# liuzuxin/FSRL

Measured on AMD Instinct MI355X. Metric: policy-updates/sec (PPO-Lagrangian update(), SafetyCarCircle-v0 shape, 256x256 MLP, 20k-step buffer), higher is better.
Workload: dtype f32; 1 GPU; configs[1] PPO-Lag update: repeat 4, clip 0.5, KL stop off, batch 256, N=20000 (20x1000), obs 8/act 2, 256x256; seeds_per_gpu=1, parallelism=independent agents x1

## Files before the change

### fsrl_amd/csrc/common.hpp

```cpp
#pragma once
#include <hip/hip_runtime.h>
#include <stdint.h>

#include "../../include/fsrl_hip.h"

#define FSRL_MAX_NETS (1 + FSRL_MAX_CRITICS)
#define FSRL_TILE_M 16
#define FSRL_DOW 32
#define FSRL_MAX_OBS 128
#define FSRL_MAX_ACT 16
#define FSRL_W1_LDS 16
#define FSRL_RD 64
#define FSRL_RD_LOGP 16
#define FSRL_RD_ADV 17
#define FSRL_RD_RET 21
#define FSRL_RD_VOLD 25
#define FSRL_RD_MEAN 32
#define FSRL_RD_STD 48

typedef float f32x4 __attribute__((ext_vector_type(4)));
typedef float f32x2 __attribute__((ext_vector_type(2)));

struct NetOff {
    int sigma;
// ... 33 lines not shown
    float rescale;
    float lam[FSRL_MAX_CRITICS];
    float eps_clip, dual_clip, vf_coef, max_action, max_grad_norm, target_kl;
    int norm_adv, use_lagrangian;
    float lr, beta1, beta2, adam_eps;
    float one_minus_b1, one_minus_b2;
    double kl_thresh;
    float step_size;
    float bc2_sqrt;
    int value_clip;
    int fuse_adam;
    int xcd_pair;
    int dbg_phase;
};
#ifdef FSRL_PROBES
#define FSRL_PROBE(sa, n) ((sa).dbg_phase == (n))
#define FSRL_TS(buf, k) do { if ((buf) && threadIdx.x == 0) (buf)[(size_t)blockIdx.x * 16 + (k)] = __builtin_readcyclecounter(); } while (0)
#else
#define FSRL_PROBE(sa, n) false
#define FSRL_TS(buf, k) do { } while (0)
#endif

__device__ __forceinline__ void ppo_adam_math(const float g, float& m, float& v, float& p, const PpoStepArgs& sa) {
#pragma clang fp contract(off)
    m = fmaf(sa.one_minus_b1, g - m, m);
    v = v * sa.beta2;
    v = fmaf(sa.one_minus_b2 * g, g, v);
    const float denom = sqrtf(v) / sa.bc2_sqrt + sa.adam_eps;
    p = p + (-sa.step_size * m) / denom;
}

struct CtrlBlock {
    int stopped_after;
    int pad;
    double kl_sum;
    float last_grad_norm;
    float pad2;
};

__device__ __forceinline__ f32x4 mfma_16x16x4(float a, float b, f32x4 c) {
    return __builtin_amdgcn_mfma_f32_16x16x4f32(a, b, c, 0, 0, 0);
}

__device__ __forceinline__ f32x4 mfma_4x4x1(float a, float b, f32x4 c) {
    return __builtin_amdgcn_mfma_f32_4x4x1f32(a, b, c, 0, 0, 0);
}

__device__ __forceinline__ void store4_next(float* p, const f32x4 v) {
    asm volatile("global_store_dwordx4 %0, %1, off sc1\n\ts_nop 1" ::"v"(p), "v"(v) : "memory");
}
#ifdef FSRL_FB_PLAIN_STORES
__device__ __forceinline__ void store4_fb(float* p, const f32x4 v) { *reinterpret_cast<f32x4*>(p) = v; }
#else
__device__ __forceinline__ void store4_fb(float* p, const f32x4 v) { store4_next(p, v); }
#endif

__host__ __device__ __forceinline__ unsigned div_magic(const int d) { return d > 1 ? 0xFFFFFFFFu / (unsigned)d + 1u : 0u; }
__device__ __forceinline__ int div_by_magic(const unsigned e, const unsigned magic) { return magic ? (int)__umulhi(e, magic) : (int)e; }

#ifndef WG3_NO_BUFFER
typedef unsigned wg3_u32x4 __attribute__((ext_vector_type(4)));
struct Wg3Buf { __amdgpu_buffer_rsrc_t r; };
__device__ __forceinline__ Wg3Buf wg3_buf(const float* base) {
    Wg3Buf b; b.r = __builtin_amdgcn_make_buffer_rsrc(const_cast<float*>(base), 0, 0x7FFFFFFF, 0x00020000); return b;
}
__device__ __forceinline__ Wg3Buf wg3_buf_here(const float* base) {
    unsigned long long p = (unsigned long long)base;
// ... 37 lines not shown
```

### fsrl_amd/csrc/fsrl_hip.hip

```cpp
#include <hip/hip_runtime.h>

#include <climits>
#include <cstddef>
#include <cmath>
#include <cstdarg>
#include <cstdio>
#include <cstdlib>
#include <cstring>
#include <algorithm>
#include <functional>
#include <queue>
#include <string>
#include <vector>

#include "kernels_misc.hpp"
#include "kernels_mlp.hpp"
#include "kernels_fb.hpp"
#include "kernels_fbco.hpp"
#include "kernels_wgrad2.hpp"
#include "kernels_wgrad3.hpp"
#include "kernels_layered.hpp"
#include "kernels_focops_group.hpp"

static thread_local std::string g_err;
// ... 55 lines not shown
    struct CommState* comm = nullptr;
    int device = 0;
    hipStream_t compute = nullptr, side = nullptr;
    ModelDesc md{};
    std::vector<TensorMap> tmap;
    int h1 = 0, h2 = 0;
    int64_t n_api = 0;
    int n_dev = 0;
    int n_alloc = 0;
    float *P = nullptr, *M = nullptr, *V = nullptr, *G = nullptr;
    int64_t adam_t = 0;
    CtrlBlock* ctrl = nullptr;
    CtrlBlock* h_ctrl = nullptr;
    bool verdict_pending = false;

    int64_t sub_size = 0, maxsize = 0;
    float* mbstat = nullptr; size_t mbstat_cap = 0;
    double* d_rms = nullptr;
    double* ret64 = nullptr; int64_t ret64_cap = 0;
    int64_t alloc_rows = 0;
    int active_envs = 0;
    std::vector<EnvBook> env;
    std::vector<uint8_t> h_flags;
    StorePtrs st{};
    static constexpr int STAGE_CAP = 4096;
    Staging stage[2];
    int cur_stage = 0;
    hipEvent_t store_ready = nullptr;

    BatchPtrs b{};
    int* d_indices = nullptr; uint8_t* d_end = nullptr; int* d_seg = nullptr;
    int* h_indices = nullptr; uint8_t* h_end = nullptr; int* h_seg = nullptr;
    float *values = nullptr, *vnext = nullptr, *advs = nullptr, *rets = nullptr, *logp_old = nullptr;
    int64_t N = 0;
    int n_seg = 0;
    bool batch_ready = false;

    int batch_size = 0, mbp_max = 0, n_tiles_max = 0;
    float *A1 = nullptr, *A2 = nullptr, *D1 = nullptr, *D2 = nullptr, *DO = nullptr;
    float *obs_p = nullptr, *rd_p = nullptr;
    float *statp = nullptr, *gsq_part = nullptr;
    int *d_perm = nullptr, *h_perm = nullptr;
    int *d_mbstart = nullptr, *d_mbsize = nullptr, *h_mbplan = nullptr;
    size_t mb_cap = 0;
    std::vector<int> mb_start, mb_size;
    float* d_stats = nullptr; int64_t stats_cap = 0;
    int64_t n_steps = 0;
    int pass_index = 0;
    double lagr[FSRL_MAX_CRITICS] = {0, 0, 0, 0};
    double rescaling = 1.0;
    bool in_update = false;

    void* scratch = nullptr; size_t scratch_bytes = 0;

    bool profiling = false;
    hipEvent_t ev_a = nullptr, ev_b = nullptr, ev_c = nullptr;
    std::vector<hipEvent_t> k_ev;
    size_t k_ev_used = 0;
    double t_process_ms = 0, t_learn_ms = 0, t_fwdbwd_ms = 0, t_fwdbwd_raw_ms = 0;
    int64_t n_fwdbwd = 0;
    uint64_t rng[4] = {0x9E3779B97F4A7C15ull, 0xBF58476D1CE4E5B9ull, 0x94D049BB133111EBull, 1};
    uint64_t shuffle_rng[4] = {0xD6E8FEB86659FD93ull, 0xA0761D6478BD642Full, 0xE7037ED1A0B428DBull, 2};
    struct Parts { int stride = 0; float* p = nullptr; size_t floats = 0; } parts[3];
    float* wg_parts = nullptr;
    int n_cus = 256;
    bool wgrad_xcd = false;
// ... 227 lines not shown
    for (int net = 0; net < md.n_nets; ++net) {
        const NetOff& no = md.net[net];
        for (int n = 0; n < H; ++n)
            for (int k = 0; k < H; ++k) v[(size_t)no.W2f + w2f_index(H, n, k)] = v[(size_t)no.W2 + (size_t)n * H + k];
    }
}

extern "C" int fsrl_ctx_destroy(fsrl_ctx* c) {
    if (!c) return 0;
    (void)hipSetDevice(c->device);
    pactor_release(c);
    (void)hipDeviceSynchronize();
    if (c->group) group_detach(c);
    if (c->sac_group) sac_group_detach(c);
    if (c->cvpo_group) cvpo_group_detach(c);
    comm_free(c);
    tr_free(c);
    sac_free(c);
    foc_free(c);
    lay_free(c);
    if (c->h_actor) (void)hipHostFree(c->h_actor);
    if (c->h_done) (void)hipHostFree(c->h_done);
    if (c->h_pa) (void)hipHostFree(c->h_pa);
    if (c->mbstat) (void)hipFree(c->mbstat);
    if (c->d_rms) (void)hipFree(c->d_rms);
    if (c->ret64) (void)hipFree(c->ret64);
    if (c->mu_old) (void)hipFree(c->mu_old);
    if (c->sigma_old) (void)hipFree(c->sigma_old);
    if (c->snap) (void)hipFree(c->snap);
    void* dptrs[] = {c->P, c->M, c->V, c->G, c->ctrl, c->st.obs, c->st.obs_next, c->st.act, c->st.rew,
                     c->st.cost, c->st.flags, c->b.obs, c->b.obs_next, c->b.act, c->b.rew, c->b.cost,
                     c->b.flags, c->d_indices, c->d_end, c->d_seg, c->values, c->vnext, c->advs,
                     c->rets, c->logp_old, c->A1, c->A2, c->D1, c->D2, c->DO, c->obs_p, c->rd_p, c->statp,
                     c->gsq_part, c->d_perm, c->d_mbstart, c->d_mbsize, c->d_stats,
                     c->scratch};
    for (void* p : dptrs) if (p) (void)hipFree(p);
    for (auto& pp : c->parts) if (pp.p) (void)hipFree(pp.p);
    void* hptrs[] = {c->h_ctrl, c->h_indices, c->h_end, c->h_seg, c->h_perm, c->h_mbplan};
    for (void* p : hptrs) if (p) (void)hipHostFree(p);
    for (auto& s : c->stage) {
        if (s.h) (void)hipHostFree(s.h);
        if (s.d) (void)hipFree(s.d);
        if (s.done) (void)hipEventDestroy(s.done);
    }
    for (hipEvent_t e : {c->store_ready, c->ev_a, c->ev_b, c->ev_c, c->perm_copied}) if (e) (void)hipEventDestroy(e);
    for (hipEvent_t e : c->k_ev) (void)hipEventDestroy(e);
    if (c->compute) (void)hipStreamDestroy(c->compute);
    if (c->side) (void)hipStreamDestroy(c->side);
    delete c;
    return 0;
}

extern "C" int fsrl_ctx_create(int device_id, const fsrl_config* cfg, fsrl_ctx** out) {
    CHECK_ARG(cfg && out, "null argument");
    CHECK_ARG(cfg->algo == FSRL_ALGO_PPO_LAG || cfg->algo == FSRL_ALGO_SAC_LAG || cfg->algo == FSRL_ALGO_CPO ||
                  cfg->algo == FSRL_ALGO_TRPO_LAG || cfg->algo == FSRL_ALGO_FOCOPS, "unknown algo %d", cfg->algo);
    CHECK_ARG(cfg->obs_dim >= 1 && cfg->obs_dim <= FSRL_MAX_OBS, "obs_dim must be in [1,%d]", FSRL_MAX_OBS);
    CHECK_ARG(cfg->act_dim >= 1 && cfg->act_dim <= FSRL_MAX_ACT, "act_dim must be in [1,%d]", FSRL_MAX_ACT);
    CHECK_ARG(cfg->n_hidden >= 0 && cfg->n_hidden <= FSRL_MAX_HIDDEN, "n_hidden must be in [0, %d]", FSRL_MAX_HIDDEN);
    bool layered = false;
    int n_hid1 = cfg->hidden1, n_hid2 = cfg->hidden2;
    if (cfg->n_hidden > 0) {
        CHECK_ARG(cfg->hidden1 == 0 && cfg->hidden2 == 0, "give hidden_sizes[n_hidden] or hidden1 / hidden2, not both");
        for (int l = 0; l < cfg->n_hidden; ++l)
            CHECK_ARG(cfg->hidden_sizes[l] >= 1 && cfg->hidden_sizes[l] <= FSRL_MAX_WIDTH, "hidden_sizes[%d] = %d outside [1, %d]", l,
                      cfg->hidden_sizes[l], FSRL_MAX_WIDTH);
        if (cfg->n_hidden == 2 && cfg->hidden_sizes[0] <= 256 && cfg->hidden_sizes[1] <= 256 && !cfg->force_layered) {
// ... 53 lines not shown
    TRY(hipStreamCreateWithFlags(&c->compute, hipStreamNonBlocking));
    TRY(hipStreamCreateWithFlags(&c->side, hipStreamNonBlocking));
    const size_t pb = (size_t)c->n_dev * sizeof(float);
    TRY(hipMalloc(&c->P, (size_t)c->n_alloc * sizeof(float))); TRY(hipMemsetAsync(c->P, 0, (size_t)c->n_alloc * sizeof(float), c->compute));
    TRY(hipMalloc(&c->M, pb)); TRY(hipMalloc(&c->V, pb)); TRY(hipMalloc(&c->G, pb));
    TRY(hipMemsetAsync(c->M, 0, pb, c->compute)); TRY(hipMemsetAsync(c->V, 0, pb, c->compute)); TRY(hipMemsetAsync(c->G, 0, pb, c->compute));
    TRY(hipMalloc(&c->ctrl, sizeof(CtrlBlock)));
    if (cfg->rew_norm) {
        TRY(hipMalloc(&c->d_rms, 3 * FSRL_MAX_CRITICS * sizeof(double)));
        double init[3 * FSRL_MAX_CRITICS];
        for (int i = 0; i < FSRL_MAX_CRITICS; ++i) { init[3 * i] = 0.0; init[3 * i + 1] = 1.0; init[3 * i + 2] = 0.0; }
        TRY(hipMemcpy(c->d_rms, init, sizeof(init), hipMemcpyHostToDevice));
    }
    TRY(hipHostMalloc(&c->h_ctrl, sizeof(CtrlBlock)));
    c->sub_size = (cfg->buffer_size + cfg->env_num - 1) / cfg->env_num;
    c->maxsize = c->sub_size * cfg->env_num;
    c->alloc_rows = c->maxsize + cfg->env_num; c->active_envs = cfg->env_num;
    c->env.resize(cfg->env_num);
    c->h_flags.assign((size_t)c->alloc_rows, 0);
    const size_t ms = (size_t)c->alloc_rows;
    const int Do = cfg->obs_dim, Da = cfg->act_dim;
    TRY(hipMalloc(&c->st.obs, ms * Do * 4)); TRY(hipMalloc(&c->st.obs_next, ms * Do * 4));
    TRY(hipMalloc(&c->st.act, ms * Da * 4)); TRY(hipMalloc(&c->st.rew, ms * 8));
    TRY(hipMalloc(&c->st.cost, ms * 8)); TRY(hipMalloc(&c->st.flags, ms));
    TRY(hipMalloc(&c->b.obs, ms * Do * 4)); TRY(hipMalloc(&c->b.obs_next, ms * Do * 4));
    TRY(hipMalloc(&c->b.act, ms * Da * 4)); TRY(hipMalloc(&c->b.rew, ms * 8));
    TRY(hipMalloc(&c->b.cost, ms * 8)); TRY(hipMalloc(&c->b.flags, ms));
    TRY(hipMalloc(&c->d_indices, ms * 4)); TRY(hipMalloc(&c->d_end, ms)); TRY(hipMalloc(&c->d_seg, (ms + 2) * 4));
    TRY(hipHostMalloc(&c->h_indices, ms * 4)); TRY(hipHostMalloc(&c->h_end, ms)); TRY(hipHostMalloc(&c->h_seg, (ms + 2) * 4));
    const int C = cfg->n_critics;
    TRY(hipMalloc(&c->values, ms * C * 4)); TRY(hipMalloc(&c->vnext, ms * C * 4));
    TRY(hipMalloc(&c->advs, ms * C * 4)); TRY(hipMalloc(&c->rets, ms * C * 4));
    TRY(hipMalloc(&c->logp_old, ms * 4));
    TRY(hipMalloc(&c->d_perm, ms * 4)); TRY(hipHostMalloc(&c->h_perm, ms * 4));
    TRY(hipMalloc(&c->obs_p, (ms + 32) * Do * 4)); TRY(hipMemsetAsync(c->obs_p, 0, (ms + 32) * Do * 4, c->compute));
    TRY(hipMalloc(&c->rd_p, (ms + 32) * FSRL_RD * 4)); TRY(hipMemsetAsync(c->rd_p, 0, (ms + 32) * FSRL_RD * 4, c->compute));
    TRY(hipStreamSynchronize(c->compute));
    for (auto& s : c->stage) {
        const size_t k = fsrl_ctx::STAGE_CAP;
        TRY(hipHostMalloc(&s.h, k * stage_rec_bytes(Do, Da)));
        TRY(hipMalloc(&s.d, k * stage_rec_bytes(Do, Da)));
        TRY(hipEventCreateWithFlags(&s.done, hipEventDisableTiming));
    }
    TRY(hipEventCreateWithFlags(&c->store_ready, hipEventDisableTiming));
    TRY(hipEventCreate(&c->ev_a)); TRY(hipEventCreate(&c->ev_b)); TRY(hipEventCreate(&c->ev_c));
    TRY(hipEventCreateWithFlags(&c->perm_copied, hipEventDisableTiming));
    CtrlBlock init{INT_MAX, 0, 0.0, 0.0f, 0.0f};
    TRY(hipMemcpy(c->ctrl, &init, sizeof(init), hipMemcpyHostToDevice));
#undef TRY
    *out = c;
    return 0;
}

extern "C" int fsrl_sync(fsrl_ctx* c) {
    CHECK_ARG(c, "null ctx");
    ENTER_DEV(c);
    HIPCHK(hipStreamSynchronize(c->side));
    HIPCHK(hipStreamSynchronize(c->compute));
    return 0;
}

extern "C" int64_t fsrl_param_count(const fsrl_ctx* c) { return c ? c->n_api : 0; }

static int copy_flat(fsrl_ctx* c, float* dev, float* host_out, const float* host_in, int64_t n) {
    CHECK_ARG(n == c->n_api, "expected %lld parameters, got %lld", (long long)c->n_api, (long long)n);
    ENTER_DEV(c);
// ... 229 lines not shown
    }
    return 0;
}

extern "C" int fsrl_store_read(fsrl_ctx* c, const int64_t* indices, int64_t n, float* obs_out, float* act_out,
                               double* rew_out, double* cost_out, uint8_t* terminated_out, uint8_t* truncated_out,
                               float* obs_next_out) {
    CHECK_ARG(c && (indices || n == 0), "null argument");
    CHECK_ARG(n >= 0 && n <= c->maxsize, "bad row count");
    if (n == 0) return 0;
    ENTER_DEV(c);
    int rc = join_store(c);
    if (rc) return rc;
    const size_t N = (size_t)n, Do = (size_t)c->cfg.obs_dim, Da = (size_t)c->cfg.act_dim;
    auto al = [](size_t x) { return (x + 255) / 256 * 256; };
    const size_t o_idx = 0, o_end = o_idx + al(N * 4), o_obs = o_end + al(N), o_nxt = o_obs + al(N * Do * 4),
                 o_act = o_nxt + al(N * Do * 4), o_rew = o_act + al(N * Da * 4), o_cost = o_rew + al(N * 8),
                 o_fl = o_cost + al(N * 8), total = o_fl + al(N);
    rc = ensure_scratch(c, total);
    if (rc) return rc;
    std::vector<int> idx(N);
    for (size_t i = 0; i < N; ++i) {
        CHECK_ARG(indices[i] >= 0 && indices[i] < c->maxsize, "index %lld out of range", (long long)indices[i]);
        idx[i] = (int)indices[i];
    }
    char* base = (char*)c->scratch;
    hipStream_t s = c->compute;
    HIPCHK(hipMemcpyAsync(base + o_idx, idx.data(), N * 4, hipMemcpyHostToDevice, s));
    HIPCHK(hipMemsetAsync(base + o_end, 0, N, s));
    BatchPtrs b{(float*)(base + o_obs), (float*)(base + o_nxt), (float*)(base + o_act), (double*)(base + o_rew),
                (double*)(base + o_cost), (uint8_t*)(base + o_fl)};
    const size_t work = N * (2 * Do + Da + 1);
    hipLaunchKernelGGL(batch_gather_kernel, dim3((int)std::min<size_t>(2048, (work + 255) / 256)), dim3(256), 0, s, c->st, b,
                       (const int*)(base + o_idx), (const uint8_t*)(base + o_end), (int)n, (int)Do, (int)Da);
    HIPCHK(hipGetLastError());
    std::vector<uint8_t> fl(N);
    if (obs_out) HIPCHK(hipMemcpyAsync(obs_out, b.obs, N * Do * 4, hipMemcpyDeviceToHost, s));
    if (obs_next_out) HIPCHK(hipMemcpyAsync(obs_next_out, b.obs_next, N * Do * 4, hipMemcpyDeviceToHost, s));
    if (act_out) HIPCHK(hipMemcpyAsync(act_out, b.act, N * Da * 4, hipMemcpyDeviceToHost, s));
    if (rew_out) HIPCHK(hipMemcpyAsync(rew_out, b.rew, N * 8, hipMemcpyDeviceToHost, s));
    if (cost_out) HIPCHK(hipMemcpyAsync(cost_out, b.cost, N * 8, hipMemcpyDeviceToHost, s));
    HIPCHK(hipMemcpyAsync(fl.data(), b.flags, N, hipMemcpyDeviceToHost, s));
    HIPCHK(hipStreamSynchronize(s));
    for (size_t i = 0; i < N; ++i) {
        if (terminated_out) terminated_out[i] = fl[i] & 1;
        if (truncated_out) truncated_out[i] = (fl[i] >> 1) & 1;
    }
    return 0;
}

template <typename F>
static int dispatch_H(int H, F&& f) {
    switch (H) {
        case 64: return f(std::integral_constant<int, 64>());
        case 128: return f(std::integral_constant<int, 128>());
        case 256: return f(std::integral_constant<int, 256>());
    }
    return fail(FSRL_EINVAL, "unsupported hidden width %d", H);
}

static int launch_infer(fsrl_ctx* c, const InferArgs& ia, int jobs_y, hipStream_t s) {
    const int tiles = (ia.N + 15) / 16;
    if (tiles == 0) return 0;
    if (c->lay) return lay_infer(c, ia, jobs_y, s);
    return dispatch_H(c->cfg.hidden, [&](auto hc) {
        constexpr int H = decltype(hc)::value;
        const int gx = std::min(tiles, std::max(1, c->n_cus / jobs_y));
        hipLaunchKernelGGL(mlp_infer_kernel<H>, dim3(gx, jobs_y), dim3(4 * H), 0, s, c->P, c->md, ia);
        HIPCHK(hipGetLastError());
        return 0;
    });
}

struct SacState;
static bool ctx_is_replay(const fsrl_ctx* c) { return c->cfg.algo == FSRL_ALGO_SAC_LAG; }
static int sac_actor_launch(fsrl_ctx* c, const float* h_obs, float* h_raw, int k);
static void sac_actor_finish(fsrl_ctx* c, const float* h_raw, int k, float* mu_out, float* sigma_out);
static int sac_raw_cols(const fsrl_ctx* c);
static bool sac_squashes(fsrl_ctx* c);
static bool sac_actor_resident_args(fsrl_ctx* c, const float** P, const ModelDesc** md);

struct PaLayout { unsigned long long* bell; unsigned* done; unsigned* state; float* obs; float* mu; float* sp; };
static PaLayout pa_layout(const fsrl_ctx* c) {
    char* b = (char*)c->h_pa;
    PaLayout l;
    l.bell = (unsigned long long*)b; l.done = (unsigned*)(b + 16); l.state = (unsigned*)(b + 32);
    l.obs = (float*)(b + 64);
    l.mu = l.obs + (size_t)c->pa_cap * c->cfg.obs_dim;
    l.sp = l.mu + (size_t)c->pa_cap * 2 * c->cfg.act_dim;
    return l;
}

static bool pactor_ok(const fsrl_ctx* c, int k) {
    const int blocks = std::min(PACTOR_BLOCKS, std::max(1, (c->cfg.env_num + 15) / 16));
    if (!(c->pa_on && !c->no_spin && !c->lay && !c->group && k >= 1 && k <= 16 * blocks)) return false;
    if (c->cfg.algo != FSRL_ALGO_SAC_LAG) return true;
    const float* P; const ModelDesc* md;
    return sac_actor_resident_args(const_cast<fsrl_ctx*>(c), &P, &md);
}

static void pactor_release(fsrl_ctx* c) {
// ... 528 lines not shown
```

### fsrl_amd/csrc/host_ppo.inc

```
static int launch_gae(fsrl_ctx* c);
static void split_plan(int n, int B, std::vector<int>& st, std::vector<int>& sz) {
    st.clear(); sz.clear();
    const bool merge = (n % B) > 0;
    for (int i = 0; i < n; i += B) {
        if (merge && i + 2 * B >= n) { st.push_back(i); sz.push_back(n - i); break; }
        st.push_back(i); sz.push_back(std::min(B, n - i));
    }
}

static int ensure_ppo_buffers(fsrl_ctx* c, int B) {
    const int mbp = round_up(2 * B, 32);
    if (mbp <= c->mbp_max) return 0;
    HIPCHK(hipStreamSynchronize(c->compute));
    for (float** p : {&c->A1, &c->A2, &c->D1, &c->D2, &c->DO, &c->statp, &c->gsq_part})
        if (*p) { HIPCHK(hipFree(*p)); *p = nullptr; }
    const int H = c->cfg.hidden, nn = c->md.n_nets;
    const size_t act = (size_t)nn * mbp * H * 4;
    HIPCHK(hipMalloc(&c->A1, act)); HIPCHK(hipMalloc(&c->A2, act));
    HIPCHK(hipMalloc(&c->D1, act)); HIPCHK(hipMalloc(&c->D2, act));
    HIPCHK(hipMalloc(&c->DO, (size_t)nn * mbp * FSRL_DOW * 4));
    HIPCHK(hipMalloc(&c->statp, (size_t)(mbp / 4) * nn * 4 * 4));
    HIPCHK(hipMalloc(&c->gsq_part, (size_t)std::max(wg_grid(H, nn), c->n_dev / 256 + 2) * 4));
    c->mbp_max = mbp;
    c->n_tiles_max = mbp / 16;
// ... 21 lines not shown
    for (int i = 0; i < FSRL_MAX_CRITICS; ++i) c->lagr[i] = 0.0;
    if (c->cfg.use_lagrangian && C > 1) {
        CHECK_ARG(lagrangians, "lags and values length must be equal");
        for (int i = 0; i < C - 1; ++i) c->lagr[i] = lagrangians[i];
    }
    c->rescaling = rescaling;
    c->batch_size = batch_size;
    const int64_t n = sample0(c, c->h_indices, c->h_end);
    c->N = n;
    if (n_out) *n_out = n;
    c->n_steps = 0;
    c->pass_index = 0;
    c->in_update = true;
    c->verdict_pending = false;
    c->t_fwdbwd_ms = 0; c->n_fwdbwd = 0; c->k_ev_used = 0;
    CtrlBlock init{INT_MAX, 0, 0.0, 0.0f, 0.0f};
    *c->h_ctrl = init;
    hipStream_t s = c->compute;
    HIPCHK(hipMemcpyAsync(c->ctrl, c->h_ctrl, sizeof(CtrlBlock), hipMemcpyHostToDevice, s));
    if (n == 0) { c->batch_ready = true; return 0; }
    int nseg = 0;
    c->h_seg[nseg++] = 0;
    for (int64_t i = 0; i + 1 < n; ++i) if (c->h_end[i]) c->h_seg[nseg++] = (int)i + 1;
    c->h_seg[nseg] = (int)n;
    HIPCHK(hipEventRecord(c->ev_a, s));
    HIPCHK(hipMemcpyAsync(c->d_indices, c->h_indices, (size_t)n * 4, hipMemcpyHostToDevice, s));
    HIPCHK(hipMemcpyAsync(c->d_end, c->h_end, (size_t)n, hipMemcpyHostToDevice, s));
    HIPCHK(hipMemcpyAsync(c->d_seg, c->h_seg, (size_t)(nseg + 1) * 4, hipMemcpyHostToDevice, s));
    const int Do = c->cfg.obs_dim, Da = c->cfg.act_dim;
    {
        const size_t work = (size_t)n * (2 * Do + Da + 1);
        const int blocks = (int)std::min<size_t>(2048, (work + 255) / 256);
        hipLaunchKernelGGL(batch_gather_kernel, dim3(blocks), dim3(256), 0, s, c->st, c->b, c->d_indices,
                           c->d_end, (int)n, Do, Da);
        HIPCHK(hipGetLastError());
    }
    InferArgs ia{};
    ia.obs = c->b.obs; ia.obs_next = c->b.obs_next; ia.act = c->b.act; ia.flags = c->b.flags;
    ia.values = c->values; ia.vnext = c->vnext; ia.logp_old = c->logp_old; ia.mu_out = nullptr;
    if (c->cfg.algo == FSRL_ALGO_FOCOPS) {
        if (!c->mu_old) {
            HIPCHK(hipMalloc(&c->mu_old, (size_t)c->alloc_rows * Da * 4));
            HIPCHK(hipMalloc(&c->sigma_old, FSRL_MAX_ACT * 4));
        }
        ia.mu_out = c->mu_old;
        HIPCHK(hipMemcpyAsync(c->sigma_old, c->P + c->md.net[0].sigma, (size_t)Da * 4, hipMemcpyDeviceToDevice, s));
    }
    ia.N = (int)n; ia.C = C; ia.max_action = c->cfg.max_action;
    rc = launch_infer(c, ia, 2 * C + 1, s);
    if (rc) return rc;
    c->n_seg = nseg;
    rc = launch_gae(c);
    if (rc) return rc;
    HIPCHK(hipEventRecord(c->ev_b, s));
    split_plan((int)n, batch_size, c->mb_start, c->mb_size);
    const int bs_rows = (int)std::min<int64_t>(batch_size, std::max<int64_t>(n, 1));
    rc = c->lay ? lay_ensure_mb(c, bs_rows) : ensure_ppo_buffers(c, bs_rows);
    if (rc) return rc;
    const size_t nmb = c->mb_start.size();
    if (nmb > c->mb_cap) {
        HIPCHK(hipStreamSynchronize(s));
        if (c->d_mbstart) HIPCHK(hipFree(c->d_mbstart));
        if (c->d_mbsize) HIPCHK(hipFree(c->d_mbsize));
        if (c->h_mbplan) HIPCHK(hipHostFree(c->h_mbplan));
        c->d_mbstart = c->d_mbsize = nullptr; c->h_mbplan = nullptr;
        const size_t cap = nmb * 2;
        HIPCHK(hipMalloc(&c->d_mbstart, cap * 4)); HIPCHK(hipMalloc(&c->d_mbsize, cap * 4));
        HIPCHK(hipHostMalloc(&c->h_mbplan, cap * 2 * 4));
        c->mb_cap = cap;
    }
    memcpy(c->h_mbplan, c->mb_start.data(), nmb * 4);
    memcpy(c->h_mbplan + c->mb_cap, c->mb_size.data(), nmb * 4);
    HIPCHK(hipMemcpyAsync(c->d_mbstart, c->h_mbplan, nmb * 4, hipMemcpyHostToDevice, s));
    HIPCHK(hipMemcpyAsync(c->d_mbsize, c->h_mbplan + c->mb_cap, nmb * 4, hipMemcpyHostToDevice, s));
    c->batch_ready = true;
    return 0;
}


static int launch_gae(fsrl_ctx* c) {
    GaeArgs ga{};
    ga.values = c->values; ga.vnext = c->vnext; ga.rew = c->b.rew; ga.cost = c->b.cost; ga.flags = c->b.flags;
    ga.seg_start = c->d_seg; ga.advs = c->advs; ga.rets = c->rets; ga.adv64 = nullptr; ga.N = (int)c->N;
    ga.gamma = c->cfg.gamma; ga.gl = c->cfg.gamma * c->cfg.gae_lambda;
    if (c->cfg.rew_norm) {
        if (c->ret64_cap < c->N) {
            HIPCHK(hipStreamSynchronize(c->compute));
            if (c->ret64) HIPCHK(hipFree(c->ret64));
            c->ret64 = nullptr;
            HIPCHK(hipMalloc(&c->ret64, (size_t)c->cfg.n_critics * c->alloc_rows * 8));
            c->ret64_cap = c->alloc_rows;
        }
        ga.rms = c->d_rms; ga.ret64 = c->ret64;
    }
    hipLaunchKernelGGL(gae_kernel, dim3(c->n_seg, c->cfg.n_critics), dim3(64), 0, c->compute, ga);
    HIPCHK(hipGetLastError());
    if (c->cfg.rew_norm) {
        hipLaunchKernelGGL(ret_rms_update_kernel, dim3(c->cfg.n_critics), dim3(1024), 0, c->compute, c->ret64, c->d_rms,
                           (int)c->N);
        HIPCHK(hipGetLastError());
    }
    return 0;
}

static int ppo_recompute_advantages(fsrl_ctx* c) {
    const int C = c->cfg.n_critics;
    InferArgs ia{};
    ia.obs = c->b.obs; ia.obs_next = c->b.obs_next; ia.act = nullptr; ia.flags = c->b.flags;
    ia.values = c->values; ia.vnext = c->vnext; ia.logp_old = nullptr; ia.mu_out = nullptr;
    ia.N = (int)c->N; ia.C = C; ia.max_action = c->cfg.max_action;
    int rc = launch_infer(c, ia, 2 * C, c->compute);
    if (rc) return rc;
    return launch_gae(c);
}

static int ensure_stats(fsrl_ctx* c, int64_t steps) {
    if (steps <= c->stats_cap) return 0;
    int64_t cap = std::max<int64_t>(steps, c->stats_cap * 2);
    cap = std::max<int64_t>(cap, 1024);
    float* nw = nullptr;
    HIPCHK(hipMalloc(&nw, (size_t)cap * FSRL_PPO_NSTATS * 4));
    if (c->d_stats) {
        HIPCHK(hipStreamSynchronize(c->compute));
        HIPCHK(hipMemcpy(nw, c->d_stats, (size_t)c->stats_cap * FSRL_PPO_NSTATS * 4, hipMemcpyDeviceToDevice));
        HIPCHK(hipFree(c->d_stats));
    }
    c->d_stats = nw;
    c->stats_cap = cap;
    return 0;
}

static int ppo_pass_prepare(fsrl_ctx* c, const int64_t* perm, uint64_t seed) {
    const int n = (int)c->N;
    hipStream_t s = c->compute;
    const int C = c->cfg.n_critics;
    if (c->cfg.recompute_adv && c->pass_index > 0 &&
        (c->cfg.algo == FSRL_ALGO_PPO_LAG || c->cfg.algo == FSRL_ALGO_FOCOPS)) {
        int rc0 = ppo_recompute_advantages(c);
        if (rc0) return rc0;
    }
    c->perm_tmp.resize((size_t)n);
    if (perm) {
        std::vector<uint8_t> seen((size_t)n, 0);
// ... 278 lines not shown
```

### fsrl_amd/csrc/kernels_misc.hpp

```cpp
#pragma once
#include "common.hpp"

struct StorePtrs {
    float* obs;
    float* obs_next;
    float* act;
    double* rew;
    double* cost;
    uint8_t* flags;
};

__global__ void store_scatter_kernel(StorePtrs st, const uint8_t* __restrict__ recs, const int rec, int k, int Do, int Da) {
    const int per = 2 * Do + Da + 1;
    for (int e = blockIdx.x * blockDim.x + threadIdx.x; e < k * per; e += gridDim.x * blockDim.x) {
        const int row = e / per, f = e - row * per;
        const uint8_t* r = recs + (size_t)row * rec;
        const size_t dst = (size_t)*reinterpret_cast<const int*>(r + 16);
        const float* x = reinterpret_cast<const float*>(r + 24);
        if (f < Do) st.obs[dst * Do + f] = x[f];
        else if (f < 2 * Do) st.obs_next[dst * Do + (f - Do)] = x[f];
        else if (f < 2 * Do + Da) st.act[dst * Da + (f - 2 * Do)] = x[f];
        else {
            st.rew[dst] = *reinterpret_cast<const double*>(r);
            st.cost[dst] = *reinterpret_cast<const double*>(r + 8);
            st.flags[dst] = (uint8_t)*reinterpret_cast<const uint32_t*>(r + 20);
        }
    }
}

struct BatchPtrs {
    float* obs; float* obs_next; float* act; double* rew; double* cost; uint8_t* flags;
};

__global__ void batch_gather_kernel(StorePtrs st, BatchPtrs b, const int* __restrict__ indices,
                                    const uint8_t* __restrict__ end_flag, int n, int Do, int Da) {
    const int per = 2 * Do + Da + 1;
    for (size_t e = (size_t)blockIdx.x * blockDim.x + threadIdx.x; e < (size_t)n * per;
         e += (size_t)gridDim.x * blockDim.x) {
        const int row = (int)(e / per), f = (int)(e - (size_t)row * per);
        const size_t src = (size_t)indices[row];
        if (f < Do) b.obs[(size_t)row * Do + f] = st.obs[src * Do + f];
        else if (f < 2 * Do) b.obs_next[(size_t)row * Do + (f - Do)] = st.obs_next[src * Do + (f - Do)];
        else if (f < 2 * Do + Da) b.act[(size_t)row * Da + (f - 2 * Do)] = st.act[src * Da + (f - 2 * Do)];
        else {
            b.rew[row] = st.rew[src];
            b.cost[row] = st.cost[src];
            b.flags[row] = (uint8_t)((st.flags[src] & 3) | (end_flag[row] ? 4 : 0));
        }
    }
}

struct GaeArgs {
    const float* values;
    const float* vnext;
    const double* rew;
    const double* cost;
    const uint8_t* flags;
    const int* seg_start;
    float* advs;
    float* rets;
    double* adv64;
    int N;
    double gamma, gl;
    const double* rms;
    double* ret64;
};
#define FSRL_RMS_EPS 1e-8

__device__ __forceinline__ double readlane_f64(double x, int l) {
    const int lo = __builtin_amdgcn_readlane(__double2loint(x), l);
    const int hi = __builtin_amdgcn_readlane(__double2hiint(x), l);
    return __hiloint2double(hi, lo);
}

__global__ __launch_bounds__(64) void gae_kernel(const GaeArgs a) {
#pragma clang fp contract(off)
    const int seg = blockIdx.x, c = blockIdx.y, lane = threadIdx.x;
    const int s = a.seg_start[seg], e = a.seg_start[seg + 1];
    const float* __restrict__ v = a.values + (size_t)c * a.N;
    const float* __restrict__ vn = a.vnext + (size_t)c * a.N;
    const double* __restrict__ met = (c == 0) ? a.rew : a.cost;
    const double scale = a.rms ? sqrt(a.rms[3 * c + 1] + FSRL_RMS_EPS) : 1.0;
    double g = 0.0;
    for (int base = e - 64; base > s - 64; base -= 64) {
        const int idx = base + lane;
        const bool ok = idx >= s;
        double delta = 0.0, disc = 0.0, vv = 0.0;
        if (ok) {
            vv = (double)v[idx];
            double vnx = (double)vn[idx];
            if (a.rms) { vv = vv * scale; vnx = vnx * scale; }
            const double t0 = vnx * a.gamma;
            const double t1 = met[idx] + t0;
            delta = t1 - vv;
            disc = (1.0 - ((a.flags[idx] & 4) ? 1.0 : 0.0)) * a.gl;
        }
        double res = 0.0;
#pragma unroll
        for (int t = 63; t >= 0; --t) {
            const double dt = readlane_f64(delta, t);
            const double ct = readlane_f64(disc, t);
            const double prod = ct * g;
            g = dt + prod;
            if (lane == t) res = g;
        }
        if (ok) {
            const size_t o = (size_t)c * a.N + idx;
            a.advs[o] = (float)res;
            double ret = res + vv;
            if (a.rms) { ret = ret / scale; a.ret64[o] = ret; }
            a.rets[o] = (float)ret;
            if (a.adv64) a.adv64[o] = res;
        }
    }
}

__global__ __launch_bounds__(1024) void ret_rms_update_kernel(const double* __restrict__ ret64, double* __restrict__ rms,
                                                              const int N) {
    __shared__ double sh[16];
    __shared__ double bc;
    const int c = blockIdx.x, tid = threadIdx.x;
    const double* __restrict__ x = ret64 + (size_t)c * N;
    auto block_sum = [&](double v) {
// ... 225 lines not shown
```

### fsrl_amd/csrc/kernels_mlp.hpp

```cpp
#pragma once
#include "common.hpp"

__host__ __device__ constexpr int tile_rows(int R) { return R > 16 ? R : 16; }

template <int H, int ROWS = 16>
struct TileSmem {
    static constexpr int LD = H + 4;
    static constexpr int XK = (ROWS > 16) ? 64 : FSRL_MAX_OBS;
    float xT[XK * ROWS];
    float h1[ROWS * LD];
    float h2[ROWS * LD];
    float d2[ROWS * LD];
    float out[ROWS * FSRL_MAX_ACT];
    float dout[ROWS * FSRL_DOW];
    float rd[ROWS * FSRL_RD];
    float st[ROWS * 4];
    float w3[FSRL_MAX_ACT * H];
    float b1[H], b2[H], b3[FSRL_MAX_ACT], sig[FSRL_MAX_ACT];
    float w1[H * FSRL_W1_LDS];
};

template <int H>
struct TileGeom {
    static constexpr int NT = 4 * H;
// ... 256 lines not shown
            }
            __syncthreads();
            return;
        }
    }
    for (int idx = wave; idx < R * no.out; idx += WAVES) {
        const int i = idx / no.out, o = idx - i * no.out;
        const float* w3 = &sm.w3[o * H];
        float s = 0.0f;
#pragma unroll
        for (int k = lane; k < H; k += 64) s = fmaf(sm.h2[i * LD + k], w3[k], s);
        s = wave_sum(s);
        if (lane == 0) sm.out[i * FSRL_MAX_ACT + o] = s + sm.b3[o];
    }
    __syncthreads();
}

struct InferArgs {
    const float* obs;
    const float* obs_next;
    const float* act;
    const uint8_t* flags;
    float* values;
    float* vnext;
    float* logp_old;
    float* mu_out;
    int N, C;
    float max_action;
    float* raw_out;
    int raw_cols;
    float* sigma_param_out;
    unsigned* done;
    unsigned seq;
};

#define LOG_SQRT_2PI 0.9189385332046727f

template <int H>
__global__ __launch_bounds__(4 * H) void mlp_infer_kernel(const float* __restrict__ P,
                                                         const ModelDesc md, const InferArgs a) {
    __shared__ TileSmem<H> sm;
    constexpr int NT = TileGeom<H>::NT;
    constexpr int NX = TileStage<H>::NX;
    const int tid = threadIdx.x;
    const int job = blockIdx.y;
    const int C = a.C;
    const bool is_actor = (job == 2 * C);
    const int net = is_actor ? 0 : 1 + (C > 0 ? job % C : 0);
    const bool use_next = (!is_actor) && job >= C;
    const NetOff no = md.net[net];
    const int Do = md.Do;
    const int n_tiles = (a.N + 15) >> 4;
    const unsigned magic = div_magic(Do);
    const float* __restrict__ X = use_next ? a.obs_next : a.obs;
    int tile = blockIdx.x;
    int row0 = tile * 16;
    int n_valid = min(16, a.N - row0);
    TileStage<H> stg;
    stg.issue(P, no, Do, md.Da, X + (size_t)row0 * Do, nullptr, n_valid, tid);
    FwdW2Frag<H> wf;
    wf.load(P + no.W2f, tid >> 6, tid & 63);
    stg.commit(sm, no, Do, tid);
    while (true) {
        const int ntile = tile + gridDim.x;
        const int nrow0 = ntile * 16, nn_valid = min(16, a.N - nrow0);
        float xn[NX];
        if (ntile < n_tiles) {
#pragma unroll
            for (int u = 0; u < NX; ++u) {
                const int e = tid + u * NT;
                xn[u] = (e < nn_valid * Do) ? X[(size_t)nrow0 * Do + e] : 0.0f;
            }
        }
        __syncthreads();
        tile_forward<H>(sm, P, no, Do, tid, wf);
        if (a.sigma_param_out && is_actor && tile == 0 && tid < md.Da && no.sigma >= 0) a.sigma_param_out[tid] = sm.sig[tid];
        if (a.raw_out) {
            for (int e = tid; e < n_valid * a.raw_cols; e += NT) {
                const int i = e / a.raw_cols, o = e - i * a.raw_cols;
                a.raw_out[(size_t)(row0 + i) * a.raw_cols + o] = sm.out[i * FSRL_MAX_ACT + o];
            }
        } else if (tid < n_valid) {
            const int r = row0 + tid;
            if (!is_actor) {
                float v = sm.out[tid * FSRL_MAX_ACT];
                const int c = (C > 0) ? job % C : 0;
                if (use_next) {
                    if (a.flags[r] & 1) v = 0.0f;
                    a.vnext[(size_t)c * a.N + r] = v;
                } else {
                    a.values[(size_t)c * a.N + r] = v;
                }
            } else {
                float logp = 0.0f;
                for (int d = 0; d < md.Da; ++d) {
                    const float x = sm.out[tid * FSRL_MAX_ACT + d];
                    const float mu = md.unbounded ? x : a.max_action * tanhf(x);
                    const float sig = expf(sm.sig[d]);
                    if (a.mu_out) a.mu_out[(size_t)r * md.Da + d] = mu;
                    if (a.act) {
                        const float diff = a.act[(size_t)r * md.Da + d] - mu;
                        logp += -(diff * diff) / (2.0f * sig * sig) - logf(sig) - LOG_SQRT_2PI;
                    }
                }
                if (a.logp_old) a.logp_old[r] = logp;
            }
        }
        if (ntile >= n_tiles) break;
        __syncthreads();
#pragma unroll
        for (int u = 0; u < NX; ++u) {
            const int e = tid + u * NT;
            if (e < 16 * Do) { const int i = div_by_magic((unsigned)e, magic), k = e - i * Do; sm.xT[k * 16 + i] = xn[u]; }
        }
        tile = ntile; row0 = nrow0; n_valid = nn_valid;
    }
    if (a.done) {
        if (tid < min(NT, max(256, (16 * a.raw_cols + 63) & ~63))) __atomic_thread_fence(__ATOMIC_RELEASE);
        __syncthreads();
        if (tid == 0) __hip_atomic_store(a.done + blockIdx.x, a.seq, __ATOMIC_RELAXED, __HIP_MEMORY_SCOPE_SYSTEM);
    }
}

#define PACTOR_BLOCKS 4
struct PActorArgs {
    const float* obs;
    float* mu_out;
    float* sigma_param_out;
    const unsigned long long* bell;
    unsigned* done;
    unsigned* state;
    unsigned gen, last_seq;
    unsigned long long timeout_ticks;
    float max_action;
    int raw_cols;
};
#define PACTOR_EXIT 0xFFFFFFFFu

template <int H, bool RAW>
__global__ __launch_bounds__(4 * H) void actor_resident_kernel(const float* __restrict__ P, const ModelDesc md, const PActorArgs a) {
    __shared__ TileSmem<H> sm;
    __shared__ unsigned k_s, seq_s;
    __shared__ unsigned last_s;
    constexpr int NT = TileGeom<H>::NT;
    constexpr int NX = TileStage<H>::NX;
    const int tid = threadIdx.x, blk = blockIdx.x;
// ... 953 lines not shown
```

Measured before the change: 129.0 updates/s.

## Skip critic inference on obs_next rows chained to the next row's obs

The batch gather kernel now marks each row whose obs_next bit-equals the following row's obs, and appends every other row to a compact list. Critic inference on obs_next runs only over the listed rows through a remapped 1D grid. For chained rows the GAE kernel takes V(s') from values[idx+1], or zero on terminal. This removes most of the duplicate next-state critic forward passes, at the cost of an extra comparison pass, an atomic list build and gathered input loads in the listed tiles.

```diff
diff --git a/fsrl_amd/csrc/common.hpp b/fsrl_amd/csrc/common.hpp
--- a/fsrl_amd/csrc/common.hpp
+++ b/fsrl_amd/csrc/common.hpp
@@ -89,7 +89,7 @@
 
 struct CtrlBlock {
     int stopped_after;
-    int pad;
+    int n_unchained;
     double kl_sum;
     float last_grad_norm;
     float pad2;
diff --git a/fsrl_amd/csrc/fsrl_hip.hip b/fsrl_amd/csrc/fsrl_hip.hip
--- a/fsrl_amd/csrc/fsrl_hip.hip
+++ b/fsrl_amd/csrc/fsrl_hip.hip
@@ -111,6 +111,8 @@
     int* d_indices = nullptr; uint8_t* d_end = nullptr; int* d_seg = nullptr;
     int* h_indices = nullptr; uint8_t* h_end = nullptr; int* h_seg = nullptr;
     float *values = nullptr, *vnext = nullptr, *advs = nullptr, *rets = nullptr, *logp_old = nullptr;
+    uint8_t* d_chain = nullptr;
+    int* d_unch = nullptr;
     int64_t N = 0;
     int n_seg = 0;
     bool batch_ready = false;
@@ -404,7 +406,7 @@
                      c->st.cost, c->st.flags, c->b.obs, c->b.obs_next, c->b.act, c->b.rew, c->b.cost,
                      c->b.flags, c->d_indices, c->d_end, c->d_seg, c->values, c->vnext, c->advs,
                      c->rets, c->logp_old, c->A1, c->A2, c->D1, c->D2, c->DO, c->obs_p, c->rd_p, c->statp,
-                     c->gsq_part, c->d_perm, c->d_mbstart, c->d_mbsize, c->d_stats,
+                     c->gsq_part, c->d_perm, c->d_mbstart, c->d_mbsize, c->d_stats, c->d_chain, c->d_unch,
                      c->scratch};
     for (void* p : dptrs) if (p) (void)hipFree(p);
     for (auto& pp : c->parts) if (pp.p) (void)hipFree(pp.p);
@@ -524,6 +526,7 @@
     TRY(hipMalloc(&c->values, ms * C * 4)); TRY(hipMalloc(&c->vnext, ms * C * 4));
     TRY(hipMalloc(&c->advs, ms * C * 4)); TRY(hipMalloc(&c->rets, ms * C * 4));
     TRY(hipMalloc(&c->logp_old, ms * 4));
+    TRY(hipMalloc(&c->d_chain, ms)); TRY(hipMalloc(&c->d_unch, ms * 4));
     TRY(hipMalloc(&c->d_perm, ms * 4)); TRY(hipHostMalloc(&c->h_perm, ms * 4));
     TRY(hipMalloc(&c->obs_p, (ms + 32) * Do * 4)); TRY(hipMemsetAsync(c->obs_p, 0, (ms + 32) * Do * 4, c->compute));
     TRY(hipMalloc(&c->rd_p, (ms + 32) * FSRL_RD * 4)); TRY(hipMemsetAsync(c->rd_p, 0, (ms + 32) * FSRL_RD * 4, c->compute));
@@ -819,7 +822,8 @@
                 (double*)(base + o_cost), (uint8_t*)(base + o_fl)};
     const size_t work = N * (2 * Do + Da + 1);
     hipLaunchKernelGGL(batch_gather_kernel, dim3((int)std::min<size_t>(2048, (work + 255) / 256)), dim3(256), 0, s, c->st, b,
-                       (const int*)(base + o_idx), (const uint8_t*)(base + o_end), (int)n, (int)Do, (int)Da);
+                       (const int*)(base + o_idx), (const uint8_t*)(base + o_end), (int)n, (int)Do, (int)Da, (uint8_t*)nullptr,
+                       (int*)nullptr, (int*)nullptr);
     HIPCHK(hipGetLastError());
     std::vector<uint8_t> fl(N);
     if (obs_out) HIPCHK(hipMemcpyAsync(obs_out, b.obs, N * Do * 4, hipMemcpyDeviceToHost, s));
@@ -853,7 +857,13 @@
     return dispatch_H(c->cfg.hidden, [&](auto hc) {
         constexpr int H = decltype(hc)::value;
         const int gx = std::min(tiles, std::max(1, c->n_cus / jobs_y));
-        hipLaunchKernelGGL(mlp_infer_kernel<H>, dim3(gx, jobs_y), dim3(4 * H), 0, s, c->P, c->md, ia);
+        if (ia.list) {
+            InferArgs la = ia;
+            const int n_full = jobs_y - ia.C;
+            la.gx_list = gx; la.gx_full = std::min(tiles, std::max(1, c->n_cus / n_full));
+            hipLaunchKernelGGL(mlp_infer_kernel<H>, dim3(ia.C * la.gx_list + n_full * la.gx_full), dim3(4 * H), 0, s, c->P, c->md, la);
+        } else
+            hipLaunchKernelGGL(mlp_infer_kernel<H>, dim3(gx, jobs_y), dim3(4 * H), 0, s, c->P, c->md, ia);
         HIPCHK(hipGetLastError());
         return 0;
     });
diff --git a/fsrl_amd/csrc/host_ppo.inc b/fsrl_amd/csrc/host_ppo.inc
--- a/fsrl_amd/csrc/host_ppo.inc
+++ b/fsrl_amd/csrc/host_ppo.inc
@@ -77,7 +77,7 @@
         const size_t work = (size_t)n * (2 * Do + Da + 1);
         const int blocks = (int)std::min<size_t>(2048, (work + 255) / 256);
         hipLaunchKernelGGL(batch_gather_kernel, dim3(blocks), dim3(256), 0, s, c->st, c->b, c->d_indices,
-                           c->d_end, (int)n, Do, Da);
+                           c->d_end, (int)n, Do, Da, c->lay ? nullptr : c->d_chain, c->d_unch, &c->ctrl->n_unchained);
         HIPCHK(hipGetLastError());
     }
     InferArgs ia{};
@@ -92,6 +92,7 @@
         HIPCHK(hipMemcpyAsync(c->sigma_old, c->P + c->md.net[0].sigma, (size_t)Da * 4, hipMemcpyDeviceToDevice, s));
     }
     ia.N = (int)n; ia.C = C; ia.max_action = c->cfg.max_action;
+    if (!c->lay) { ia.list = c->d_unch; ia.list_n = &c->ctrl->n_unchained; }
     rc = launch_infer(c, ia, 2 * C + 1, s);
     if (rc) return rc;
     c->n_seg = nseg;
@@ -128,6 +129,7 @@
     ga.values = c->values; ga.vnext = c->vnext; ga.rew = c->b.rew; ga.cost = c->b.cost; ga.flags = c->b.flags;
     ga.seg_start = c->d_seg; ga.advs = c->advs; ga.rets = c->rets; ga.adv64 = nullptr; ga.N = (int)c->N;
     ga.gamma = c->cfg.gamma; ga.gl = c->cfg.gamma * c->cfg.gae_lambda;
+    ga.chain = c->lay ? nullptr : c->d_chain;
     if (c->cfg.rew_norm) {
         if (c->ret64_cap < c->N) {
             HIPCHK(hipStreamSynchronize(c->compute));
@@ -154,6 +156,7 @@
     ia.obs = c->b.obs; ia.obs_next = c->b.obs_next; ia.act = nullptr; ia.flags = c->b.flags;
     ia.values = c->values; ia.vnext = c->vnext; ia.logp_old = nullptr; ia.mu_out = nullptr;
     ia.N = (int)c->N; ia.C = C; ia.max_action = c->cfg.max_action;
+    if (!c->lay) { ia.list = c->d_unch; ia.list_n = &c->ctrl->n_unchained; }
     int rc = launch_infer(c, ia, 2 * C, c->compute);
     if (rc) return rc;
     return launch_gae(c);
diff --git a/fsrl_amd/csrc/kernels_misc.hpp b/fsrl_amd/csrc/kernels_misc.hpp
--- a/fsrl_amd/csrc/kernels_misc.hpp
+++ b/fsrl_amd/csrc/kernels_misc.hpp
@@ -33,7 +33,8 @@
 };
 
 __global__ void batch_gather_kernel(StorePtrs st, BatchPtrs b, const int* __restrict__ indices,
-                                    const uint8_t* __restrict__ end_flag, int n, int Do, int Da) {
+                                    const uint8_t* __restrict__ end_flag, int n, int Do, int Da,
+                                    uint8_t* __restrict__ chain, int* __restrict__ unch_list, int* __restrict__ unch_count) {
     const int per = 2 * Do + Da + 1;
     for (size_t e = (size_t)blockIdx.x * blockDim.x + threadIdx.x; e < (size_t)n * per;
          e += (size_t)gridDim.x * blockDim.x) {
@@ -48,11 +49,27 @@
             b.flags[row] = (uint8_t)((st.flags[src] & 3) | (end_flag[row] ? 4 : 0));
         }
     }
+    if (chain == nullptr) return;
+    const int lane = threadIdx.x & 63;
+    const int n_waves = (int)((gridDim.x * blockDim.x) >> 6);
+    for (int row = (int)((blockIdx.x * blockDim.x + threadIdx.x) >> 6); row < n; row += n_waves) {
+        bool differs = row + 1 >= n;
+        if (!differs) {
+            const unsigned* __restrict__ nx = reinterpret_cast<const unsigned*>(st.obs_next + (size_t)indices[row] * Do);
+            const unsigned* __restrict__ ob = reinterpret_cast<const unsigned*>(st.obs + (size_t)indices[row + 1] * Do);
+            for (int k = lane; k < Do; k += 64) differs = differs || nx[k] != ob[k];
+        }
+        const bool unchained = __ballot(differs) != 0ull;
+        if (lane == 0) {
+            chain[row] = unchained ? 0 : 1;
+            if (unchained) unch_list[atomicAdd(unch_count, 1)] = row;
+        }
+    }
 }
 
 struct GaeArgs {
     const float* values;
-    const float* vnext;
+    float* vnext;
     const double* rew;
     const double* cost;
     const uint8_t* flags;
@@ -64,6 +81,7 @@
     double gamma, gl;
     const double* rms;
     double* ret64;
+    const uint8_t* chain;
 };
 #define FSRL_RMS_EPS 1e-8
 
@@ -77,8 +95,8 @@
 #pragma clang fp contract(off)
     const int seg = blockIdx.x, c = blockIdx.y, lane = threadIdx.x;
     const int s = a.seg_start[seg], e = a.seg_start[seg + 1];
-    const float* __restrict__ v = a.values + (size_t)c * a.N;
-    const float* __restrict__ vn = a.vnext + (size_t)c * a.N;
+    const float* v = a.values + (size_t)c * a.N;
+    float* vn = a.vnext + (size_t)c * a.N;
     const double* __restrict__ met = (c == 0) ? a.rew : a.cost;
     const double scale = a.rms ? sqrt(a.rms[3 * c + 1] + FSRL_RMS_EPS) : 1.0;
     double g = 0.0;
@@ -88,7 +106,12 @@
         double delta = 0.0, disc = 0.0, vv = 0.0;
         if (ok) {
             vv = (double)v[idx];
-            double vnx = (double)vn[idx];
+            float vn32;
+            if (a.chain && a.chain[idx]) {
+                vn32 = (a.flags[idx] & 1) ? 0.0f : v[idx + 1];
+                vn[idx] = vn32;
+            } else vn32 = vn[idx];
+            double vnx = (double)vn32;
             if (a.rms) { vv = vv * scale; vnx = vnx * scale; }
             const double t0 = vnx * a.gamma;
             const double t1 = met[idx] + t0;
diff --git a/fsrl_amd/csrc/kernels_mlp.hpp b/fsrl_amd/csrc/kernels_mlp.hpp
--- a/fsrl_amd/csrc/kernels_mlp.hpp
+++ b/fsrl_amd/csrc/kernels_mlp.hpp
@@ -312,9 +312,21 @@
     float* sigma_param_out;
     unsigned* done;
     unsigned seq;
+    const int* list;
+    const int* list_n;
+    int gx_list, gx_full;
 };
 
 #define LOG_SQRT_2PI 0.9189385332046727f
+
+template <int NT>
+__device__ __forceinline__ void infer_stage_listed(float* __restrict__ xT, const float* __restrict__ X, const int* __restrict__ rows,
+                                                   const int nv, const int Do, const unsigned magic, const int tid) {
+    for (int e = tid; e < 16 * Do; e += NT) {
+        const int i = div_by_magic((unsigned)e, magic), k = e - i * Do;
+        xT[k * 16 + i] = (i < nv) ? X[(size_t)rows[i] * Do + k] : 0.0f;
+    }
+}
 
 template <int H>
 __global__ __launch_bounds__(4 * H) void mlp_infer_kernel(const float* __restrict__ P,
@@ -323,29 +335,41 @@
     constexpr int NT = TileGeom<H>::NT;
     constexpr int NX = TileStage<H>::NX;
     const int tid = threadIdx.x;
-    const int job = blockIdx.y;
     const int C = a.C;
+    int job = blockIdx.y, bx = blockIdx.x, stride = gridDim.x;
+    if (a.list) {
+        const int n_listed = C * a.gx_list;
+        if ((int)blockIdx.x < n_listed) { job = C + blockIdx.x / a.gx_list; bx = blockIdx.x % a.gx_list; stride = a.gx_list; }
+        else {
+            const int id = blockIdx.x - n_listed, j = id / a.gx_full;
+            job = j < C ? j : 2 * C; bx = id - j * a.gx_full; stride = a.gx_full;
+        }
+    }
     const bool is_actor = (job == 2 * C);
     const int net = is_actor ? 0 : 1 + (C > 0 ? job % C : 0);
     const bool use_next = (!is_actor) && job >= C;
+    const bool listed = use_next && a.list != nullptr;
     const NetOff no = md.net[net];
     const int Do = md.Do;
-    const int n_tiles = (a.N + 15) >> 4;
+    const int n_rows = listed ? min(max(*a.list_n, 0), a.N) : a.N;
+    const int n_tiles = (n_rows + 15) >> 4;
+    if (bx >= n_tiles) return;
     const unsigned magic = div_magic(Do);
     const float* __restrict__ X = use_next ? a.obs_next : a.obs;
-    int tile = blockIdx.x;
+    int tile = bx;
     int row0 = tile * 16;
-    int n_valid = min(16, a.N - row0);
+    int n_valid = min(16, n_rows - row0);
     TileStage<H> stg;
-    stg.issue(P, no, Do, md.Da, X + (size_t)row0 * Do, nullptr, n_valid, tid);
+    stg.issue(P, no, Do, md.Da, listed ? X : X + (size_t)row0 * Do, nullptr, listed ? 0 : n_valid, tid);
     FwdW2Frag<H> wf;
     wf.load(P + no.W2f, tid >> 6, tid & 63);
     stg.commit(sm, no, Do, tid);
+    if (listed) infer_stage_listed<NT>(sm.xT, X, a.list + row0, n_valid, Do, magic, tid);
     while (true) {
-        const int ntile = tile + gridDim.x;
-        const int nrow0 = ntile * 16, nn_valid = min(16, a.N - nrow0);
+        const int ntile = tile + stride;
+        const int nrow0 = ntile * 16, nn_valid = min(16, n_rows - nrow0);
         float xn[NX];
-        if (ntile < n_tiles) {
+        if (!listed && ntile < n_tiles) {
 #pragma unroll
             for (int u = 0; u < NX; ++u) {
                 const int e = tid + u * NT;
@@ -361,7 +385,7 @@
                 a.raw_out[(size_t)(row0 + i) * a.raw_cols + o] = sm.out[i * FSRL_MAX_ACT + o];
             }
         } else if (tid < n_valid) {
-            const int r = row0 + tid;
+            const int r = listed ? a.list[row0 + tid] : row0 + tid;
             if (!is_actor) {
                 float v = sm.out[tid * FSRL_MAX_ACT];
                 const int c = (C > 0) ? job % C : 0;
@@ -388,10 +412,13 @@
         }
         if (ntile >= n_tiles) break;
         __syncthreads();
-#pragma unroll
-        for (int u = 0; u < NX; ++u) {
-            const int e = tid + u * NT;
-            if (e < 16 * Do) { const int i = div_by_magic((unsigned)e, magic), k = e - i * Do; sm.xT[k * 16 + i] = xn[u]; }
+        if (listed) infer_stage_listed<NT>(sm.xT, X, a.list + nrow0, nn_valid, Do, magic, tid);
+        else {
+#pragma unroll
+            for (int u = 0; u < NX; ++u) {
+                const int e = tid + u * NT;
+                if (e < 16 * Do) { const int i = div_by_magic((unsigned)e, magic), k = e - i * Do; sm.xT[k * 16 + i] = xn[u]; }
+            }
         }
         tile = ntile; row0 = nrow0; n_valid = nn_valid;
     }
```

Result: no change. 129.2 updates/s, median of 3 (+0.1%).
